# zj15001/PNP_ADMM_CNC_MRI

Hardware: AMD Instinct MI355X
Metric: ADMM iterations/sec on 256x256 complex64 slices (batch=512) (higher is better)
Workload: dtype f32

## Files before the change

pnp_admm_cnc_mri_amd/csrc/kernels_slice256.hip:

```cpp
#include "engine_host.h"
#include "fused_layout.h"
#include "slice_layout.h"
#include <math.h>
#include <stdio.h>
#include <stdlib.h>
#include <vector>

#ifndef SLICE_EARLY
#define SLICE_EARLY 1
#endif
#ifndef SLICE_PRIOSWAP
#define SLICE_PRIOSWAP 1
#endif
#ifndef SLICE_PRIOMASK
#define SLICE_PRIOMASK 6
#endif
#ifndef SLICE_YH_AUX
#define SLICE_YH_AUX 0
#endif
#ifndef SLICE_ST_AUX
#define SLICE_ST_AUX 0
#endif
#ifndef SLICE_RESIDENT
#define SLICE_RESIDENT 1
#endif
#ifndef SLICE_PF
#define SLICE_PF 3
#endif

namespace pnp {

__device__ c32 g_tws[256];

struct SliceArgs {
    float* z;
    float* w;
    float* x;
    const c32* Yh;
    const uint32_t* Mh;
    const c32* Ys;
    const uint32_t* Ms;
    int first, B, iters;
    int slice_xor;
    int flip;
    int state_stride;
    int yh_stride;
    float scale, c;
    ProxParams prox;
    long long* prof;
};

constexpr int RP = 18;
constexpr int REGION = 16 * RP;
constexpr int WREG = 4 * REGION;
constexpr int SL_YS = SL_BUF + REGION;
constexpr int SL_LDS = SL_YS + 256 + 32;
static_assert(SL_WAVES * WREG <= SL_BUF, "wave regions must fit in the buffer they alias");
constexpr int SL4_XB = SL_WAVES * WREG;
constexpr int SL4_YS = SL4_XB + REGION;
constexpr int SL4_RES = SL4_YS + 256 + 32;
constexpr int SL4_LDS = SL4_RES + SL_RES * 256;
static_assert(SL_BUF4 <= SL4_XB && SL4_RES % 2 == 0 && SL4_LDS * 8 <= 160 * 1024, "four-pass LDS map");
template <int PROX> constexpr bool slice_four() { return PROX == 2; }
template <int PROX> constexpr bool slice_res() { return slice_four<PROX>() && SLICE_RESIDENT; }
__device__ __forceinline__ void lds_ld4(const float* p, float (&v)[4]) {
    const float4 q = *reinterpret_cast<const float4*>(p);
    v[0] = q.x; v[1] = q.y; v[2] = q.z; v[3] = q.w;
}
__device__ __forceinline__ void lds_st4(float* p, const float (&v)[4]) { *reinterpret_cast<float4*>(p) = make_float4(v[0], v[1], v[2], v[3]); }

__device__ __forceinline__ void wave_sync() {
    __builtin_amdgcn_fence(__ATOMIC_RELEASE, "wavefront");
    __builtin_amdgcn_wave_barrier();
    __builtin_amdgcn_fence(__ATOMIC_ACQUIRE, "wavefront");
#ifdef SLICE_SYNC_SCHED_BARRIER
    __builtin_amdgcn_sched_barrier(0);
#endif
}

__device__ __forceinline__ void prio_set(int wv, int set) {
#if SLICE_PRIOSWAP
    const bool older_high = (SLICE_PRIOMASK >> set) & 1;
    if (set == 0 || (((SLICE_PRIOMASK >> set) ^ (SLICE_PRIOMASK >> (set - 1))) & 1)) {
        asm volatile("" : "+s"(wv));
        if ((wv < 4) == older_high) __builtin_amdgcn_s_setprio(1); else __builtin_amdgcn_s_setprio(0);
    }
#endif
}

__device__ __forceinline__ int opaque(int v) {
    asm volatile("" : "+v"(v));
    return v;
}
typedef unsigned int u32x4 __attribute__((ext_vector_type(4)));
typedef unsigned int u32x2 __attribute__((ext_vector_type(2)));
typedef __amdgpu_buffer_rsrc_t bufrsrc;
__device__ __forceinline__ bufrsrc make_rsrc(const void* base, unsigned bytes) {
    return __builtin_amdgcn_make_buffer_rsrc(const_cast<void*>(base), 0, (int)bytes, 0x00020000);
}
__device__ __forceinline__ void ld4(bufrsrc r, int voff, int soff, float (&v)[4]) {
    const u32x4 q = __builtin_amdgcn_raw_buffer_load_b128(r, voff, soff, 16);
    v[0] = __uint_as_float(q.x); v[1] = __uint_as_float(q.y); v[2] = __uint_as_float(q.z); v[3] = __uint_as_float(q.w);
}
__device__ __forceinline__ void st4(bufrsrc r, int voff, int soff, const float (&v)[4]) {
    u32x4 q;
    q.x = __float_as_uint(v[0]); q.y = __float_as_uint(v[1]); q.z = __float_as_uint(v[2]); q.w = __float_as_uint(v[3]);
    __builtin_amdgcn_raw_buffer_store_b128(q, r, voff + soff, 0, SLICE_ST_AUX);
}
__device__ __forceinline__ c32 ldc(bufrsrc r, int voff, int soff) {
    const u32x2 q = __builtin_amdgcn_raw_buffer_load_b64(r, voff, soff, 0);
    return mk<float>(__uint_as_float(q.x), __uint_as_float(q.y));
}
struct SliceBufs {
    bufrsrc z, w, x;
    bufrsrc yh, mh, ys, ms;
};

__device__ __forceinline__ void pin(c32& v) { asm volatile("" : "+v"(v.x), "+v"(v.y)); }
__device__ __forceinline__ void mem_fence_compiler() { asm volatile("" ::: "memory"); }

__device__ __forceinline__ float dpp_lane_xor1(float v) {
    return __int_as_float(__builtin_amdgcn_mov_dpp(__float_as_int(v), 0xB1 , 0xF, 0xF, true));
}
__device__ __forceinline__ c32 dpp_lane_xor1(c32 v) { return mk<float>(dpp_lane_xor1(v.x), dpp_lane_xor1(v.y)); }

__device__ __forceinline__ float sub_partner(float a, float b) {
    float r;
    asm("v_subrev_f32_dpp %0, %1, %2 quad_perm:[1,0,3,2] row_mask:0xf bank_mask:0xf bound_ctrl:1" : "=v"(r) : "v"(b), "v"(a));
    return r;
}
__device__ __forceinline__ float add_partner(float a, float b) {
    float r;
    asm("v_add_f32_dpp %0, %1, %2 quad_perm:[1,0,3,2] row_mask:0xf bank_mask:0xf bound_ctrl:1" : "=v"(r) : "v"(b), "v"(a));
    return r;
}

__device__ __forceinline__ float abs_plus(float a, float w) {
    float r;
    asm("v_add_f32_e64 %0, |%1|, %2" : "=v"(r) : "v"(a), "v"(w));
    return r;
}

__device__ __forceinline__ f2 sub2(f2 a, f2 b) {
    f2 r;
    asm("v_pk_add_f32 %0, %1, %2 neg_lo:[0,1] neg_hi:[0,1]" : "=v"(r) : "v"(a), "v"(b));
    return r;
}


template <bool INV>
__device__ __forceinline__ void group_fft256(c32 (&ac)[16], const c32* twl, c32* region, int t) {
    typedef float f4 __attribute__((ext_vector_type(4)));
    const f4* tw4 = reinterpret_cast<const f4*>(twl + RP * t);
    f2* reg2 = reinterpret_cast<f2*>(region);
    f2 a[16];
#pragma unroll
    for (int k = 0; k < 16; ++k) a[k] = to2(ac[k]);
    dft16_pk<INV>(a);
    mem_fence_compiler();
#pragma unroll
    for (int m = 0; m < 4; ++m) {
        const f4 q = tw4[m];
        if (m) a[2 * m] = tmul_v<INV>(a[2 * m], k2(q.x, q.y));
        a[2 * m + 1] = tmul_v<INV>(a[2 * m + 1], k2(q.z, q.w));
    }
    mem_fence_compiler();
#pragma unroll
    for (int m = 4; m < 8; ++m) {
        const f4 q = tw4[m];
        a[2 * m] = tmul_v<INV>(a[2 * m], k2(q.x, q.y));
        a[2 * m + 1] = tmul_v<INV>(a[2 * m + 1], k2(q.z, q.w));
    }
#pragma unroll
    for (int k = 0; k < 16; ++k) reg2[k * RP + t] = a[k];
    wave_sync();
    const f4* row4 = reinterpret_cast<const f4*>(reg2 + t * RP);
#pragma unroll
    for (int m = 0; m < 8; ++m) {
        const f4 q = row4[m];
        a[2 * m] = k2(q.x, q.y);
        a[2 * m + 1] = k2(q.z, q.w);
    }
    wave_sync();
    dft16_pk<INV>(a);
#pragma unroll
    for (int k = 0; k < 16; ++k) ac[k] = from2(a[k]);
}

struct RowLoads {
    float z[8][4], w[8][4];
};
__device__ __forceinline__ int row_set_offset(int set, int wv) { return (32 * set + 4 * wv) * 2048; }
constexpr int ROW_QSTRIDE = 256;

template <int PROX, bool HAS_INV, int Q0, int Q1, bool RESW = false>
__device__ __forceinline__ void issue_row_loads(const SliceBufs& b, RowLoads& L, int soff, int voff, int qbase = 0, const float* resw = nullptr) {
#pragma unroll
    for (int q = qbase + Q0; q < qbase + Q1; ++q) {
        const int vo = voff + ROW_QSTRIDE * q, so = soff;
        if (RESW) {
            ld4(b.z, vo, so, L.z[q]);
            lds_ld4(resw + 64 * q, L.w[q]);
        } else if (PROX == 3) {
            ld4(b.w, vo, so, L.w[q]);
        } else if (PROX != 0 || !HAS_INV) {
            ld4(b.z, vo, so, L.z[q]);
            ld4(b.w, vo, so, L.w[q]);
        }
    }
}

__device__ __forceinline__ f2 clamp2(f2 a, float c) {
    return k2(__builtin_amdgcn_fmed3f(a.x, -c, c), __builtin_amdgcn_fmed3f(a.y, -c, c));
}
__device__ __forceinline__ f2 fma2(f2 a, f2 b, f2 c) { return __builtin_elementwise_fma(a, b, c); }
__device__ __forceinline__ f2 splat(float v) { return k2(v, v); }
template <int PROX>
__device__ __forceinline__ void prox_pair(f2 u, f2& z, f2& w, const ProxParams& pc) {
    if (PROX == 2) {
        const f2 cz = clamp2(z, pc.ib);
        const f2 t = fma2(splat(pc.c1), z, fma2(splat(pc.c2), u, splat(pc.c3) * cz));
        z = t - clamp2(t, pc.thr);
    } else {
        z = u - clamp2(u, pc.thr);
    }
    w = u - z;
}

template <bool HAS_INV, int PROX, bool HAS_FWD, bool RESW = false>
__device__ __forceinline__ void pointwise_q(const SliceBufs& b, const ProxParams& pc, int u_first, bool last,
                                            c32& a0, c32& a1, const float (&z_)[4], const float (&w_)[4], int vs, float* resw = nullptr) {
    f2 z[2] = {k2(z_[0], z_[1]), k2(z_[2], z_[3])}, w[2] = {k2(w_[0], w_[1]), k2(w_[2], w_[3])};
#define SL_X_PLUS(a_, w_) (HAS_INV ? k2(abs_plus((a_).x, (w_).x), abs_plus((a_).y, (w_).y)) : (w_))
#define SL_ST4(buf, v) { const float q_[4] = {v[0].x, v[0].y, v[1].x, v[1].y}; st4(buf, vs, 0, q_); }
    if (PROX == 3) {
        f2 u[2];
#pragma unroll
        for (int jj = 0; jj < 2; ++jj) {
            if (!u_first) {
                asm volatile("");
                w[jj] = w[jj] - (w[jj] - clamp2(w[jj], pc.thr));
            }
            u[jj] = SL_X_PLUS(jj ? a1 : a0, w[jj]);
            z[jj] = u[jj] - clamp2(u[jj], pc.thr);
            w[jj] = u[jj] - z[jj];
        }
        if (!last) {
            SL_ST4(b.w, u);
        } else {
            SL_ST4(b.z, z);
            SL_ST4(b.w, w);
        }
    }
    if (PROX == 1 || PROX == 2) {
#pragma unroll
        for (int jj = 0; jj < 2; ++jj) prox_pair<PROX>(SL_X_PLUS(jj ? a1 : a0, w[jj]), z[jj], w[jj], pc);
        SL_ST4(b.z, z);
        if (RESW) { const float q_[4] = {w[0].x, w[0].y, w[1].x, w[1].y}; lds_st4(resw, q_); }
        else SL_ST4(b.w, w);
    }
#undef SL_ST4
#undef SL_X_PLUS
    if (HAS_FWD) {
        const f2 v0 = sub2(z[0], w[0]), v1 = sub2(z[1], w[1]);
        a0 = from2(v0);
        a1 = from2(v1);
    }
}

__device__ __forceinline__ void store_x_natural(const SliceBufs& b, const c32 (&a)[16], c32* wreg, int set, int wv, int lane) {
    const int g = lane >> 4, t = lane & 15;
    c32* region = wreg + g * REGION;
#pragma unroll
    for (int j = 0; j < 16; ++j) region[t + 16 * j] = mk<float>(fabsf(a[j].x), fabsf(a[j].y));
    wave_sync();
#pragma unroll
    for (int i = 0; i < 4; ++i) {
        const c32* cell = wreg + i * REGION + 4 * lane;
        const float4 c01 = *reinterpret_cast<const float4*>(cell);
        const float4 c23 = *reinterpret_cast<const float4*>(cell + 2);
        const int vs = 16 * lane + (2 * (32 * set + 4 * wv + i)) * 1024;
        const float xa[4] = {c01.x, c01.z, c23.x, c23.z}, xb[4] = {c01.y, c01.w, c23.y, c23.w};
        st4(b.x, vs, 0, xa);
        st4(b.x, vs + 1024, 0, xb);
    }
    wave_sync();
}

#ifndef SLICE_L1_PF
#define SLICE_L1_PF 8
#endif
template <int PROX> constexpr int row_pf() { return (PROX == 3) ? SLICE_L1_PF : SLICE_PF; }
__device__ __forceinline__ float* res_lane(float* res, int wv, int lane) { return res + sl_res_index(4 * wv + (lane >> 4), lane & 15, 0); }
template <int PROX, bool HAS_INV, bool RES = false>
__device__ __forceinline__ void row_phase_prefetch(const SliceBufs& b, RowLoads& L, int wv, int lane, float* res = nullptr) {
    issue_row_loads<PROX, HAS_INV, 0, row_pf<PROX>(), RES>(b, L, row_set_offset(0, wv), 2048 * (lane >> 4) + 16 * (lane & 15), 0, RES ? res_lane(res, wv, lane) : nullptr);
}
template <bool HAS_INV, int PROX, bool HAS_FWD, bool PRELOADED = false, bool RES = false>
__device__ __forceinline__ void row_phase(const SliceBufs& b, const ProxParams& pc, int u_first, bool last, c32 (&F)[SL_SETS][16],
                                          c32* wreg, const c32* twl, int wv, int lane, RowLoads* pre = nullptr, float* res = nullptr) {
    const int g = lane >> 4, t = lane & 15;
    c32* region = wreg + g * REGION;
    const int voff = 2048 * g + 16 * t;
    float* resw = RES ? res_lane(res, wv, lane) : nullptr;
    constexpr bool RES_LOOP = RES && HAS_INV;
    constexpr int PF = row_pf<PROX>();
    RowLoads L;
    if (PRELOADED) L = *pre;
    else issue_row_loads<PROX, HAS_INV, 0, PF, RES_LOOP>(b, L, row_set_offset(0, wv), voff, 0, resw);
#pragma unroll
    for (int set = 0; set < SL_SETS; ++set) {
        c32 (&a)[16] = F[set];
        prio_set(wv, set);
        const int soff = row_set_offset(set, wv);
        if (HAS_INV) {
            group_fft256<true>(a, twl, region, t);
        }
        if (HAS_INV && last) store_x_natural(b, a, wreg, set, wv, lane);
        const int vs = voff + soff;
#pragma unroll
        for (int q = 0; q < 8; ++q) {
            if (RES_LOOP && set == 0) {
                if (q + PF < 8) issue_row_loads<PROX, HAS_INV, 0, 1, true>(b, L, soff, voff, q + PF, resw);
                pointwise_q<HAS_INV, PROX, HAS_FWD, true>(b, pc, u_first, last, a[2 * q], a[2 * q + 1], L.z[q], L.w[q], vs + ROW_QSTRIDE * q, resw + 64 * q);
            } else {
                if (q + PF < 8) issue_row_loads<PROX, HAS_INV, 0, 1>(b, L, soff, voff, q + PF);
                if (RES && !HAS_INV && set == 0) lds_st4(resw + 64 * q, L.w[q]);
                pointwise_q<HAS_INV, PROX, HAS_FWD>(b, pc, u_first, last, a[2 * q], a[2 * q + 1], L.z[q], L.w[q], vs + ROW_QSTRIDE * q);
            }
        }
        if (set + 1 < SL_SETS) issue_row_loads<PROX, HAS_INV, 0, PF>(b, L, row_set_offset(set + 1, wv), voff);
        if (HAS_FWD) {
            group_fft256<false>(a, twl, region, t);
        }
    }
}

__device__ __forceinline__ void resident_flush(const SliceBufs& b, const float* res, int wv, int lane) {
    const float* resw = res_lane(const_cast<float*>(res), wv, lane);
    const int vs = 2048 * (lane >> 4) + 16 * (lane & 15) + row_set_offset(0, wv);
#pragma unroll
    for (int q = 0; q < 8; ++q) {
        float v[4];
        lds_ld4(resw + 64 * q, v);
        st4(b.w, vs + ROW_QSTRIDE * q, 0, v);
    }
}

#define SL_PASS0_REGS(X, t)                                                                       \
    X(0, 0, (t)) X(1, 1, (t) + 16) X(2, 2, (t) + 32) X(3, 3, (t) + 48)                              \
    X(12, 8, ((t) ? SL_M + 64 - (t) : SL_M))                                                      \
    X(13, 13, SL_M + 48 - (t)) X(14, 14, SL_M + 32 - (t)) X(15, 15, SL_M + 16 - (t))
#define SL_PASS1_REGS(X, t)                                                                       \
    X(4, 4, (t)) X(5, 5, (t) + 16) X(6, 6, (t) + 32) X(7, 7, (t) + 48)                              \
    X(8, 12, ((t) ? SL_M + 64 - (t) : SL_M))                                                      \
    X(9, 9, SL_M + 48 - (t)) X(10, 10, SL_M + 32 - (t)) X(11, 11, SL_M + 16 - (t))

#define SL_PASS4_REGS(X, t, Q)                                                                    \
    X(2 * (Q), 2 * (Q), (t)) X(2 * (Q) + 1, 2 * (Q) + 1, (t) + 16)                                  \
    X(14 - 2 * (Q), ((Q) ? 16 - 2 * (Q) : 8), ((t) ? SL_M4 + 32 - (t) : SL_M4))                   \
    X(15 - 2 * (Q), 15 - 2 * (Q), SL_M4 + 16 - (t))

__device__ __forceinline__ void lds_put(c32* p, c32 v, bool swapped) {
    float* f = reinterpret_cast<float*>(p);
    if (swapped) { f[0] = v.y; f[1] = v.x; } else { *p = v; }
}
__device__ __forceinline__ c32 lds_get(const c32* p, bool swapped) {
    const float* f = reinterpret_cast<const float*>(p);
    return swapped ? mk<float>(f[1], f[0]) : *p;
}
template <int P, bool FOUR = false>
__device__ __forceinline__ void t_store_rows(const c32 (&F)[16], c32* rp, int t) {
#define SL_T1_STORE(ja, jb, slot) { lds_put(rp + (slot), t ? F[ja] : F[jb], (ja) >= 8); }
    if (FOUR) { SL_PASS4_REGS(SL_T1_STORE, t, P) } else if (P == 0) { SL_PASS0_REGS(SL_T1_STORE, t) } else { SL_PASS1_REGS(SL_T1_STORE, t) }
#undef SL_T1_STORE
}
template <int P, bool FOUR = false>
__device__ __forceinline__ void t_load_rows(c32 (&F)[16], const c32* rp, int t) {
#define SL_T2_LOAD(ja, jb, slot) { F[ja] = lds_get(rp + (slot), (ja) >= 8); }
    if (FOUR) { SL_PASS4_REGS(SL_T2_LOAD, t, P) } else if (P == 0) { SL_PASS0_REGS(SL_T2_LOAD, t) } else { SL_PASS1_REGS(SL_T2_LOAD, t) }
#undef SL_T2_LOAD
    if (FOUR && P == 3) {
        const c32 a8 = F[8];
        F[8] = t ? a8 : F[14];
        F[14] = t ? F[14] : F[12];
        F[12] = t ? F[12] : F[10];
        F[10] = t ? F[10] : a8;
    }
    if (!FOUR && P == 1) {
        const c32 a0 = F[8];
        F[8] = t ? a0 : F[12];
        F[12] = t ? F[12] : a0;
    }
}

template <bool MAYBE_PACKED, int PITCH = SL_P>
__device__ __forceinline__ void t1_read_col(c32 (&Gs)[16], const c32* buf, int off, int odd, bool packed) {
    int off_hi = off + 64 * PITCH;
    asm volatile("" : "+v"(off_hi));
    const c32 *col = buf + off, *col_hi = buf + off_hi;
#pragma unroll
    for (int jb = 0; jb < 16; jb += 8) {
        c32 own[8];
#pragma unroll
        for (int k = 0; k < 8; ++k) own[k] = jb ? col_hi[8 * k * PITCH] : col[8 * k * PITCH];
#pragma unroll
        for (int k = 0; k < 8; ++k) {
            c32 v = mk<float>(add_partner(own[k].x, own[k].y), sub_partner(own[k].y, own[k].x));
            if (MAYBE_PACKED) {
                const float oy = dpp_lane_xor1(own[k].y);
                const c32 raw = mk<float>(odd ? oy : own[k].x, odd ? own[k].x : oy);
                v = packed ? raw : v;
            }
            Gs[jb + k] = v;
            pin(Gs[jb + k]);
        }
    }
}
template <int P>
__device__ __forceinline__ void t1_pass(const c32 (&F)[SL_SETS][16], c32 (&G)[SL_SETS][16], c32* buf, int wv, int lane) {
    const int g = lane >> 4, t = lane & 15;
#pragma unroll
    for (int set = 0; set < SL_SETS; ++set) t_store_rows<P>(F[set], buf + (32 * set + 4 * wv + g) * SL_P, t);
    __syncthreads();
#pragma unroll
    for (int h = 0; h < 2; ++h) {
        const int cc = 32 * h + 4 * wv + g, odd = t & 1;
        const int off = (t >> 1) * SL_P + cc + (odd ? SL_M : 0);
        if (P == 0 && h == 0 && wv == 0) t1_read_col<true>(G[2 * P + h], buf, off, odd, cc == 0);
        else t1_read_col<false>(G[2 * P + h], buf, off, odd, false);
    }
    __syncthreads();
}

template <bool MAYBE_PACKED, int PITCH = SL_P>
__device__ __forceinline__ void t2_write_col(const c32 (&Gs)[16], c32* buf, int off, int odd, bool packed) {
    int off_hi = off + 64 * PITCH;
    asm volatile("" : "+v"(off_hi));
    c32 *col = buf + off, *col_hi = buf + off_hi;
#pragma unroll
    for (int j = 0; j < 16; ++j) {
        const c32 own = Gs[j];
        c32 v = mk<float>(sub_partner(own.x, own.y), add_partner(own.y, own.x));
        if (MAYBE_PACKED) {
            const c32 other = dpp_lane_xor1(own);
            const c32 raw = mk<float>(odd ? own.y : own.x, odd ? other.y : other.x);
            v = packed ? raw : v;
        }
        if (j < 8) col[8 * j * PITCH] = v; else col_hi[8 * (j - 8) * PITCH] = v;
    }
}
template <int P>
__device__ __forceinline__ void t2_pass(const c32 (&G)[SL_SETS][16], c32 (&F)[SL_SETS][16], c32* buf, int wv, int lane) {
    const int g = lane >> 4, t = lane & 15;
#pragma unroll
    for (int h = 0; h < 2; ++h) {
        const int cc = 32 * h + 4 * wv + g, odd = t & 1;
        const int off = (t >> 1) * SL_P + cc + (odd ? SL_M : 0);
        if (P == 0 && h == 0 && wv == 0) t2_write_col<true>(G[2 * P + h], buf, off, odd, cc == 0);
        else t2_write_col<false>(G[2 * P + h], buf, off, odd, false);
    }
    __syncthreads();
#pragma unroll
    for (int set = 0; set < SL_SETS; ++set) t_load_rows<P>(F[set], buf + (32 * set + 4 * wv + g) * SL_P, t);
    __syncthreads();
}

template <int Q>
__device__ __forceinline__ void t1_pass4(const c32 (&F)[SL_SETS][16], c32 (&G)[SL_SETS][16], c32* buf, int wv, int lane) {
    const int g = lane >> 4, t = lane & 15;
#pragma unroll
    for (int set = 0; set < SL_SETS; ++set) t_store_rows<Q, true>(F[set], buf + (32 * set + 4 * wv + g) * SL_P4, t);
    __syncthreads();
    const int cc = 4 * wv + g, odd = t & 1;
    const int off = (t >> 1) * SL_P4 + cc + (odd ? SL_M4 : 0);
    if (Q == 0 && wv == 0) t1_read_col<true, SL_P4>(G[Q], buf, off, odd, cc == 0);
    else t1_read_col<false, SL_P4>(G[Q], buf, off, odd, false);
    __syncthreads();
}
template <int Q>
__device__ __forceinline__ void t2_pass4(const c32 (&G)[SL_SETS][16], c32 (&F)[SL_SETS][16], c32* buf, int wv, int lane) {
    const int g = lane >> 4, t = lane & 15;
    const int cc = 4 * wv + g, odd = t & 1;
    const int off = (t >> 1) * SL_P4 + cc + (odd ? SL_M4 : 0);
    if (Q == 0 && wv == 0) t2_write_col<true, SL_P4>(G[Q], buf, off, odd, cc == 0);
    else t2_write_col<false, SL_P4>(G[Q], buf, off, odd, false);
    __syncthreads();
#pragma unroll
    for (int set = 0; set < SL_SETS; ++set) t_load_rows<Q, true>(F[set], buf + (32 * set + 4 * wv + g) * SL_P4, t);
    __syncthreads();
}

struct ColLoads {
    c32 yh[16];
    uint32_t code;
};
__device__ __forceinline__ void issue_col_loads(const SliceBufs& b, ColLoads& Y, int set, int wv, int lane) {
    const int ybase = (set * 8 + wv) * 8192;
    Y.code = __builtin_amdgcn_raw_buffer_load_b32(b.mh, 4 * lane, (set * 8 + wv) * 64 * 4, 0);
#pragma unroll
    for (int jp = 0; jp < 8; ++jp) {
        const u32x4 q = __builtin_amdgcn_raw_buffer_load_b128(b.yh, 16 * lane + 1024 * (jp & 3), ybase + 4096 * (jp >> 2), SLICE_YH_AUX);
        Y.yh[2 * jp] = mk<float>(__uint_as_float(q.x), __uint_as_float(q.y));
        Y.yh[2 * jp + 1] = mk<float>(__uint_as_float(q.z), __uint_as_float(q.w));
    }
}

__device__ __forceinline__ float code_byte(unsigned m, int byte) {
    float r;
    if (byte == 0) asm("v_cvt_f32_ubyte0 %0, %1" : "=v"(r) : "v"(m));
    else if (byte == 1) asm("v_cvt_f32_ubyte1 %0, %1" : "=v"(r) : "v"(m));
    else if (byte == 2) asm("v_cvt_f32_ubyte2 %0, %1" : "=v"(r) : "v"(m));
    else asm("v_cvt_f32_ubyte3 %0, %1" : "=v"(r) : "v"(m));
    return r;
}
__device__ __forceinline__ void blend_set(c32 (&a)[16], const c32 (&yh)[16], unsigned code, float cs, float chs, float os) {
    const unsigned m[4] = {code & 0x03030303u, (code >> 2) & 0x03030303u, (code >> 4) & 0x03030303u, (code >> 6) & 0x03030303u};
#pragma unroll
    for (int j = 0; j < 16; j += 2) {
        const f2 cf = k2(code_byte(m[j & 3], j >> 2), code_byte(m[(j & 3) + 1], j >> 2));
        const f2 A2 = fma2(splat(-chs), cf, splat(os));
        a[j] = from2(fma2(A2.xx, to2(a[j]), splat(cs) * to2(yh[j])));
        a[j + 1] = from2(fma2(A2.yy, to2(a[j + 1]), splat(cs) * to2(yh[j + 1])));
    }
}

__device__ __forceinline__ void col_phase(const SliceBufs& b, float cdc, float scale, c32 (&G)[SL_SETS][16], c32* wreg, c32* ysl, const c32* twl, int wv, int lane) {
    const int g = lane >> 4, t = lane & 15;
    c32* region = wreg + g * REGION;
    const float cs = cdc * scale, chs = 0.5f * cdc * scale;
    ColLoads Y;
    issue_col_loads(b, Y, 0, wv, lane);
    if (wv == 0) {
        __builtin_amdgcn_raw_ptr_buffer_load_lds(b.ys, ysl, 16, 16 * lane, 0, 0, 0);
        __builtin_amdgcn_raw_ptr_buffer_load_lds(b.ys, ysl + 128, 16, 16 * lane, 1024, 0, 0);
        __builtin_amdgcn_raw_ptr_buffer_load_lds(b.ms, ysl + 256, 4, 4 * lane, 0, 0, 0);
    }
#pragma unroll
    for (int set = 0; set < SL_SETS; ++set) {
        c32 (&a)[16] = G[set];
        prio_set(wv, set);
        group_fft256<false>(a, twl, region, t);
        if (set == 0 && wv == 0 && g == 0) {
#pragma unroll
            for (int j = 0; j < 16; ++j) region[t + 16 * j] = a[j];
            region[256 + t] = a[0];
            wave_sync();
            const uint32_t code_b = reinterpret_cast<const uint32_t*>(ysl + 256)[t];
            const c32* mirror = region + (16 - t);
            const unsigned ma[4] = {Y.code & 0x03030303u, (Y.code >> 2) & 0x03030303u, (Y.code >> 4) & 0x03030303u, (Y.code >> 6) & 0x03030303u};
            const unsigned mb[4] = {code_b & 0x03030303u, (code_b >> 2) & 0x03030303u, (code_b >> 4) & 0x03030303u, (code_b >> 6) & 0x03030303u};
#pragma unroll
            for (int j = 0; j < 16; ++j) {
                const c32 gm = mirror[16 * (15 - j)];
                const c32 A = blend_scaled_f(unpack_a(a[j], gm), Y.yh[j], code_byte(ma[j & 3], j >> 2), cs, chs, scale);
                const c32 Bv = blend_scaled_f(unpack_b(a[j], gm), ysl[t + 16 * j], code_byte(mb[j & 3], j >> 2), cs, chs, scale);
                a[j] = repack_p(A, Bv);
            }
            wave_sync();
        } else {
            blend_set(a, Y.yh, Y.code, cs, 0.5f * chs, 0.5f * scale);
        }
        if (set + 1 < SL_SETS) issue_col_loads(b, Y, set + 1, wv, lane);
        group_fft256<true>(a, twl, region, t);
    }
}

template <int PROX>
__global__ __launch_bounds__(512) void k_slice(SliceArgs p) {
    constexpr bool FOUR = slice_four<PROX>(), RES = slice_res<PROX>();
    __shared__ __attribute__((aligned(16))) c32 lds[FOUR ? SL4_LDS : SL_LDS];
    const int tid = threadIdx.x, lane = tid & 63;
    const int wv = __builtin_amdgcn_readfirstlane(tid >> 6);
    c32* twl = lds + (FOUR ? SL4_XB : SL_BUF);
    c32* ysl = lds + (FOUR ? SL4_YS : SL_YS);
    float* res = RES ? reinterpret_cast<float*>(lds + SL4_RES) : nullptr;
    if (tid < 256) twl[RP * (tid >> 4) + (tid & 15)] = g_tws[((tid >> 4) * (tid & 15)) & 255];
    c32* wreg = lds + wv * WREG;
    __syncthreads();
    for (int sb = blockIdx.x; sb < p.B; sb += gridDim.x) {
        const int sx = ((sb ^ p.slice_xor) < p.B) ? (sb ^ p.slice_xor) : sb;
        const int slice = p.first + (p.flip ? p.B - 1 - sx : sx);
        const size_t so = (size_t)slice * p.state_stride;
        SliceBufs b;
        b.z = make_rsrc(p.z + so, 65536 * 4); b.w = make_rsrc(p.w + so, 65536 * 4); b.x = make_rsrc(p.x + (size_t)slice * 65536, 65536 * 4);
        b.yh = make_rsrc(p.Yh + (size_t)slice * p.yh_stride, YH3_SLICE * 8); b.mh = make_rsrc(p.Mh + (size_t)slice * MH3_SLICE, MH3_SLICE * 4);
        b.ys = make_rsrc(p.Ys + (size_t)slice * 256, 256 * 8); b.ms = make_rsrc(p.Ms + (size_t)slice * 16, 16 * 4);
        c32 F[SL_SETS][16];
#ifdef SLICE_PROF
        long long* prof = (p.prof && tid == 0 && sb == (int)blockIdx.x) ? p.prof + (size_t)slice * (2 + 6 * p.iters) : nullptr;
#define SL_STAMP() if (prof) *prof++ = wall_clock64()
#else
#define SL_STAMP()
#endif
        SL_STAMP();
        row_phase<false, 0, true, false, RES>(b, p.prox, 1, false, F, wreg, twl, wv, opaque(lane), nullptr, res);
        SL_STAMP();
        for (int it = 0; it < p.iters; ++it) {
            c32 G[SL_SETS][16];
            __syncthreads();
            SL_STAMP();
            if (FOUR) {
                t1_pass4<0>(F, G, lds, wv, opaque(lane));
                t1_pass4<1>(F, G, lds, wv, opaque(lane));
                t1_pass4<2>(F, G, lds, wv, opaque(lane));
                t1_pass4<3>(F, G, lds, wv, opaque(lane));
            } else {
                t1_pass<0>(F, G, lds, wv, opaque(lane));
                t1_pass<1>(F, G, lds, wv, opaque(lane));
            }
#ifdef SLICE_PROF_CLOCK
            if (prof) *prof++ = (long long)__builtin_readcyclecounter();
#else
            SL_STAMP();
#endif
            col_phase(b, p.c, p.scale, G, wreg, ysl, twl, wv, opaque(lane));
            SL_STAMP();
            __syncthreads();
            SL_STAMP();
            if (FOUR) {
                t2_pass4<0>(G, F, lds, wv, opaque(lane));
                t2_pass4<1>(G, F, lds, wv, opaque(lane));
                t2_pass4<2>(G, F, lds, wv, opaque(lane));
            } else {
                t2_pass<0>(G, F, lds, wv, opaque(lane));
            }
#if SLICE_EARLY
            RowLoads L0;
            row_phase_prefetch<PROX, true, RES>(b, L0, wv, opaque(lane), res);
#endif
            if (FOUR) t2_pass4<3>(G, F, lds, wv, opaque(lane));
            else t2_pass<1>(G, F, lds, wv, opaque(lane));
            SL_STAMP();
            const int u_first = (it == 0);
#if SLICE_EARLY
            row_phase<true, PROX, true, true, RES>(b, p.prox, u_first, it + 1 == p.iters, F, wreg, twl, wv, opaque(lane), &L0, res);
#else
            row_phase<true, PROX, true, false, RES>(b, p.prox, u_first, it + 1 == p.iters, F, wreg, twl, wv, opaque(lane), nullptr, res);
#endif
            SL_STAMP();
        }
        if (RES) resident_flush(b, res, wv, opaque(lane));
        __syncthreads();
    }
}

constexpr int SP_P = 17;
__global__ __launch_bounds__(256) void k_sprepare(const c32* y, const uint8_t* mask_bank, const int32_t* mask_id,
                                                  c32* Yh, uint32_t* Mh, c32* Ys, uint32_t* Ms, int yh_stride) {
    __shared__ c32 yd[256 * SP_P], ym[256 * SP_P];
    __shared__ uint8_t md[256 * SP_P], mm[256 * SP_P];
    const int tid = threadIdx.x, m = blockIdx.x, slice = blockIdx.y;
    const int mid = mask_id ? mask_id[slice] : 0;
    const c32* ys = y + (size_t)slice * 65536;
    const uint8_t* ms = mask_bank + (size_t)mid * 65536;
    const int ncol = (m == 8) ? 1 : 16;
#pragma unroll 4
    for (int i = 0; i < 16; ++i) {
        const int idx = tid + 256 * i, r = idx >> 4, c = idx & 15;
        if (c < ncol) {
            const int k2 = 16 * m + c, k2m = (256 - k2) & 255;
            yd[r * SP_P + c] = ys[r * 256 + k2];
            md[r * SP_P + c] = ms[r * 256 + k2];
            ym[r * SP_P + c] = ys[r * 256 + k2m];
            mm[r * SP_P + c] = ms[r * 256 + k2m];
        }
    }
    __syncthreads();
    auto entry = [&](int k1, int c, c32& yh) -> int {
        const int r2 = (256 - k1) & 255;
        const int m1 = md[k1 * SP_P + c] != 0, m2 = mm[r2 * SP_P + c] != 0;
        const c32 y1 = yd[k1 * SP_P + c], y2 = ym[r2 * SP_P + c];
        yh = mk<float>(0.5f * ((m1 ? y1.x : 0.f) + (m2 ? y2.x : 0.f)), 0.5f * ((m1 ? y1.y : 0.f) - (m2 ? y2.y : 0.f)));
        return m1 + m2;
    };
    if (m == 8) {
        c32 yh;
        const int code = entry(tid, 0, yh);
        Ys[(size_t)slice * 256 + tid] = yh;
        __shared__ int codes[256];
        codes[tid] = code;
        __syncthreads();
        if (tid < 16) {
            uint32_t v = 0;
#pragma unroll
            for (int jj = 0; jj < 16; ++jj) v |= (uint32_t)codes[tid + 16 * jj] << (2 * jj);
            Ms[slice * 16 + tid] = v;
        }
        return;
    }
    const int set = m >> 1;
#pragma unroll 4
    for (int i = 0; i < 16; ++i) {
        const int o = tid + 256 * i, blk = o >> 10, e = o & 1023;
        const int jp = e >> 7, lane = (e >> 1) & 63, j = 2 * jp + (e & 1);
        const int g = lane >> 4, t = lane & 15, wv = 4 * (m & 1) + blk;
        c32 yh;
        (void)entry(t + 16 * j, 4 * blk + g, yh);
        Yh[(size_t)slice * yh_stride + yh3_index(0, set, j, wv, lane)] = yh;
    }
    {
        const int blk = tid >> 6, lane = tid & 63, g = lane >> 4, t = lane & 15, wv = 4 * (m & 1) + blk;
        uint32_t v = 0;
#pragma unroll
        for (int j = 0; j < 16; ++j) {
            c32 yh;
            v |= (uint32_t)entry(t + 16 * j, 4 * blk + g, yh) << (2 * j);
        }
        Mh[mh3_index(slice, set, wv, lane)] = v;
    }
}

template <bool TO_SLICE>
__global__ __launch_bounds__(128) void k_state_order(const float* sz, const float* sw, float* dz, float* dw, int src_stride, int dst_stride) {
    __shared__ float tile[2][2048];
    const size_t sbase = (size_t)blockIdx.y * src_stride + (size_t)blockIdx.x * 2048, dbase = (size_t)blockIdx.y * dst_stride + (size_t)blockIdx.x * 2048;
    const float4* pz = reinterpret_cast<const float4*>(sz + sbase);
    const float4* pw = reinterpret_cast<const float4*>(sw + sbase);
    float4* qz = reinterpret_cast<float4*>(dz + dbase);
    float4* qw = reinterpret_cast<float4*>(dw + dbase);
    float4 vz[4], vw[4];
#pragma unroll
    for (int u = 0; u < 4; ++u) { vz[u] = pz[threadIdx.x + 128 * u]; vw[u] = pw[threadIdx.x + 128 * u]; }
#pragma unroll
    for (int u = 0; u < 4; ++u) {
        const int i = threadIdx.x + 128 * u, row = i >> 6, n0 = 4 * (i & 63);
        const float az[4] = {vz[u].x, vz[u].y, vz[u].z, vz[u].w}, aw[4] = {vw[u].x, vw[u].y, vw[u].z, vw[u].w};
#pragma unroll
        for (int k = 0; k < 4; ++k) {
            const int at = TO_SLICE ? (int)sl_state_index(row, n0 + k) : 4 * i + k;
            tile[0][at] = az[k];
            tile[1][at] = aw[k];
        }
    }
    __syncthreads();
#pragma unroll
    for (int u = 0; u < 4; ++u) {
        const int i = threadIdx.x + 128 * u, row = i >> 6, n0 = 4 * (i & 63);
        float oz[4], ow[4];
#pragma unroll
        for (int k = 0; k < 4; ++k) {
            const int at = TO_SLICE ? 4 * i + k : (int)sl_state_index(row, n0 + k);
            oz[k] = tile[0][at];
            ow[k] = tile[1][at];
        }
        qz[i] = make_float4(oz[0], oz[1], oz[2], oz[3]);
        qw[i] = make_float4(ow[0], ow[1], ow[2], ow[3]);
    }
}

struct Slice256 {
    int Bmax = 0, cus = 0;
    int flip = 0;
    int pad = 0, yh_pad = 0;
    float* zs = nullptr;
    float* ws = nullptr;
    c32* Yh = nullptr;
    uint32_t* Mh = nullptr;
    c32* Ys = nullptr;
    uint32_t* Ms = nullptr;
    SideQueues queues;
};

int slice256_cus(const Slice256* f) { return f && f->cus > 0 ? f->cus : 256; }

hipError_t slice256_state_order(Slice256* f, hipStream_t s, float* z, float* w, int B, bool to_slice) {
    if (B <= 0) return hipSuccess;
    if (f && f->pad > 0) {
        if (to_slice) hipLaunchKernelGGL(k_state_order<true>, dim3(32, B), dim3(128), 0, s, z, w, f->zs, f->ws, 65536, 65536 + f->pad);
        else          hipLaunchKernelGGL(k_state_order<false>, dim3(32, B), dim3(128), 0, s, f->zs, f->ws, z, w, 65536 + f->pad, 65536);
    } else {
        if (to_slice) hipLaunchKernelGGL(k_state_order<true>, dim3(32, B), dim3(128), 0, s, z, w, z, w, 65536, 65536);
        else          hipLaunchKernelGGL(k_state_order<false>, dim3(32, B), dim3(128), 0, s, z, w, z, w, 65536, 65536);
    }
    return hipGetLastError();
}

void slice256_destroy(Slice256* f) {
    if (!f) return;
    if (f->zs) (void)hipFree(f->zs);
    if (f->ws) (void)hipFree(f->ws);
    if (f->Yh) (void)hipFree(f->Yh);
    if (f->Mh) (void)hipFree(f->Mh);
    if (f->Ys) (void)hipFree(f->Ys);
    if (f->Ms) (void)hipFree(f->Ms);
    delete f;
}

Slice256* slice256_create(int Bmax, int pad_kb, int yh_pad_kb, hipError_t* err) {
    Slice256* f = new Slice256();
    f->Bmax = Bmax;
    f->pad = (pad_kb > 0 ? pad_kb : 0) * 256;
    f->yh_pad = (yh_pad_kb > 0 ? yh_pad_kb : 0) * 128;
    hipError_t e = hipMalloc((void**)&f->Yh, (size_t)Bmax * (YH3_SLICE + f->yh_pad) * sizeof(c32));
    if (e == hipSuccess && f->pad > 0) e = hipMalloc((void**)&f->zs, (size_t)Bmax * (65536 + f->pad) * sizeof(float));
    if (e == hipSuccess && f->pad > 0) e = hipMalloc((void**)&f->ws, (size_t)Bmax * (65536 + f->pad) * sizeof(float));
    if (e == hipSuccess) e = hipMalloc((void**)&f->Mh, (size_t)Bmax * MH3_SLICE * sizeof(uint32_t));
    if (e == hipSuccess) e = hipMalloc((void**)&f->Ys, (size_t)Bmax * 256 * sizeof(c32));
    if (e == hipSuccess) e = hipMalloc((void**)&f->Ms, (size_t)Bmax * 16 * sizeof(uint32_t));
    if (e == hipSuccess) e = upload_twiddle_table<float>(HIP_SYMBOL(g_tws), 256);
    if (e == hipSuccess) {
        int dev = 0;
        hipDeviceProp_t prop;
        e = hipGetDevice(&dev);
        if (e == hipSuccess) e = hipGetDeviceProperties(&prop, dev);
        if (e == hipSuccess) f->cus = prop.multiProcessorCount;
    }
    if (e != hipSuccess) {
        slice256_destroy(f);
        *err = e;
        return nullptr;
    }
    *err = hipSuccess;
    return f;
}

hipError_t slice256_prepare(Slice256* f, hipStream_t s, const float2* y, const uint8_t* mask_bank, const int32_t* mask_id, int B) {
    if (B > f->Bmax) return hipErrorInvalidValue;
    hipLaunchKernelGGL(k_sprepare, dim3(9, B), dim3(256), 0, s, reinterpret_cast<const c32*>(y), mask_bank, mask_id,
                       f->Yh, f->Mh, f->Ys, f->Ms, (int)YH3_SLICE + f->yh_pad);
    return hipGetLastError();
}

static hipError_t launch_slice(hipStream_t s, const SliceArgs& a, int prox) {
    const dim3 grid(a.B);
    if (prox == 2)      hipLaunchKernelGGL(k_slice<2>, grid, dim3(512), 0, s, a);
    else if (prox == 1) hipLaunchKernelGGL(k_slice<1>, grid, dim3(512), 0, s, a);
    else                hipLaunchKernelGGL(k_slice<3>, grid, dim3(512), 0, s, a);
    return hipGetLastError();
}

hipError_t slice256_run(Slice256* f, hipStream_t s, float* z, float* w, float* x, int B, int iters, bool cnc, float dc_c,
                        ProxParams pp, const FusedSchedule& sch) {
    if (iters <= 0) return hipSuccess;
    SliceArgs a;
    a.z = f->pad > 0 ? f->zs : z; a.w = f->pad > 0 ? f->ws : w; a.x = x; a.Yh = f->Yh;
    a.state_stride = 65536 + f->pad; a.yh_stride = (int)YH3_SLICE + f->yh_pad; a.Mh = f->Mh; a.Ys = f->Ys; a.Ms = f->Ms;
    a.first = 0; a.B = B; a.iters = iters; a.scale = 1.0f / 65536.0f; a.c = dc_c;
    a.prox = pp;
    a.prof = nullptr;
    a.flip = 0;
    a.slice_xor = sch.slice_xor;
    if (a.slice_xor < 0 || (B & (B - 1)) != 0 || a.slice_xor >= B) a.slice_xor = 0;
    const int prox = prox_kind(cnc, sch);
    int segments = sch.slice_segment > 0 ? (iters + sch.slice_segment - 1) / sch.slice_segment : 1;
    if (segments < 1) segments = 1;

    long long* d_prof = nullptr;
#ifdef SLICE_PROF
    const char* prof_path = getenv("PNP_SLICE_PROF");
#else
    const char* prof_path = nullptr;
#endif
    const LoopPlan plan = plan_slice(B, prof_path ? FusedSchedule{} : sch);
    const size_t prof_n = (size_t)B * (2 + 6 * (size_t)iters);
    if (prof_path) {
        segments = 1;
        if (hipMalloc((void**)&d_prof, prof_n * sizeof(long long)) == hipSuccess) {
            (void)hipMemsetAsync(d_prof, 0, prof_n * sizeof(long long), s);
            a.prof = d_prof;
        }
    }
    if (!prof_path && B > slice256_cus(f) && sch.slice_flip) { a.flip = f->flip; f->flip ^= 1; }
    const hipError_t e = run_parts(f->queues, s, plan, B, [&](hipStream_t sq, const Part& p) {
        hipError_t r = hipSuccess;
        int done = 0;
        for (int g = 0; g < segments && r == hipSuccess; ++g) {
            const int n = (iters - done + (segments - g) - 1) / (segments - g);
            a.first = p.first; a.B = p.count; a.iters = n;
            r = launch_slice(sq, a, prox);
            done += n;
        }
        return r;
    });
    if (d_prof) {
        std::vector<long long> h(prof_n);
        (void)hipStreamSynchronize(s);
        (void)hipMemcpy(h.data(), d_prof, prof_n * sizeof(long long), hipMemcpyDeviceToHost);
        (void)hipFree(d_prof);
        if (FILE* fo = fopen(prof_path, "wb")) {
            const int hdr[2] = {B, iters};
            fwrite(hdr, sizeof(int), 2, fo);
            fwrite(h.data(), sizeof(long long), prof_n, fo);
            fclose(fo);
        }
    }
    return e;
}

}
```

pnp_admm_cnc_mri_amd/csrc/slice_layout.h:

```cpp
#pragma once
#include <stddef.h>
#include <stdint.h>
#include "fft16.h"

namespace pnp {

constexpr int SL_P = 132;
constexpr int SL_M = 66;
constexpr int SL_BUF = 128 * SL_P;

PNP_HD int sl_pass(int k) { return (k < 64 || k > 192 || k == 128) ? 0 : 1; }
PNP_HD int sl_slot(int k) {
    if (k < 64) return k;
    if (k == 128) return SL_M;
    if (k > 192) return SL_M + 256 - k;
    if (k < 128) return k - 64;
    return SL_M + 192 - k;
}
constexpr int SL_P4 = 68;
constexpr int SL_M4 = 34;
constexpr int SL_BUF4 = 128 * SL_P4;
PNP_HD int sl_pass4(int k) { return k == 128 ? 0 : k < 128 ? (k >> 5) : ((256 - k) >> 5); }
PNP_HD int sl_slot4(int k) { return k == 128 ? SL_M4 : k < 128 ? (k & 31) : SL_M4 + ((256 - k) & 31); }
constexpr int SL_RES = 32;
PNP_HD int sl_res_index(int r, int t, int q) { return 512 * r + 64 * q + 4 * t; }

constexpr int SL_WAVES = 8, SL_SETS = 4;
PNP_HD int sl_unit(int set, int wv, int lane) { return 32 * set + 4 * wv + (lane >> 4); }

constexpr size_t YH3_SLICE = 4 * 16 * 8 * 64;
constexpr size_t MH3_SLICE = 4 * 8 * 64;
PNP_HD size_t yh3_index(int slice, int set, int j, int wv, int lane) {
    return (size_t)slice * YH3_SLICE + ((((size_t)set * 8 + wv) * 8 + (j >> 1)) * 64 + lane) * 2 + (j & 1);
}
PNP_HD size_t mh3_index(int slice, int set, int wv, int lane) { return (size_t)slice * MH3_SLICE + (((size_t)set * 8 + wv) * 64 + lane); }

PNP_HD size_t sl_state_index(int row, int n) {
    return (size_t)(row >> 1) * 512 + 64 * (n >> 5) + 4 * (n & 15) + 2 * ((n >> 4) & 1) + (row & 1);
}


}
```

Before: 10850.

## Keep more of the w state resident in LDS and registers across ADMM iterations

Generalizes the resident-w scheme from set 0 only to a per-(set, q) home map. Each w chunk lives in LDS, in registers, or in HBM, chosen by compile-time unit masks. By default two more units of set 1 go to a second LDS region and two units of set 3 are held in registers. This cuts global w load and store traffic per iteration, at the cost of extra LDS footprint and register pressure, which may reduce occupancy or cause spills.

```diff
diff --git a/pnp_admm_cnc_mri_amd/csrc/kernels_slice256.hip b/pnp_admm_cnc_mri_amd/csrc/kernels_slice256.hip
--- a/pnp_admm_cnc_mri_amd/csrc/kernels_slice256.hip
+++ b/pnp_admm_cnc_mri_amd/csrc/kernels_slice256.hip
@@ -20,9 +20,6 @@
 #endif
 #ifndef SLICE_ST_AUX
 #define SLICE_ST_AUX 0
-#endif
-#ifndef SLICE_RESIDENT
-#define SLICE_RESIDENT 1
 #endif
 #ifndef SLICE_PF
 #define SLICE_PF 3
@@ -59,7 +56,8 @@
 constexpr int SL4_XB = SL_WAVES * WREG;
 constexpr int SL4_YS = SL4_XB + REGION;
 constexpr int SL4_RES = SL4_YS + 256 + 32;
-constexpr int SL4_LDS = SL4_RES + SL_RES * 256;
+__device__ __forceinline__ int sl_lds_float(int set, int q) { return set == 0 ? sl_res_index(0, 0, q) : sl_res1_index(popc8(sl_units_lds(set) & ((1u << q) - 1)), 0, 0); }
+constexpr int SL4_LDS = SL4_RES + SL_RES * 256 + SL_NLDS1 * 1024;
 static_assert(SL_BUF4 <= SL4_XB && SL4_RES % 2 == 0 && SL4_LDS * 8 <= 160 * 1024, "four-pass LDS map");
 template <int PROX> constexpr bool slice_four() { return PROX == 2; }
 template <int PROX> constexpr bool slice_res() { return slice_four<PROX>() && SLICE_RESIDENT; }
@@ -194,13 +192,14 @@
 constexpr int ROW_QSTRIDE = 256;
 
 template <int PROX, bool HAS_INV, int Q0, int Q1, bool RESW = false>
-__device__ __forceinline__ void issue_row_loads(const SliceBufs& b, RowLoads& L, int soff, int voff, int qbase = 0, const float* resw = nullptr) {
+__device__ __forceinline__ void issue_row_loads(const SliceBufs& b, RowLoads& L, int soff, int voff, int qbase = 0, int set = 0, const float* resl = nullptr) {
 #pragma unroll
     for (int q = qbase + Q0; q < qbase + Q1; ++q) {
         const int vo = voff + ROW_QSTRIDE * q, so = soff;
-        if (RESW) {
+        const int home = RESW ? w_home(set, q) : W_HBM;
+        if (home != W_HBM) {
             ld4(b.z, vo, so, L.z[q]);
-            lds_ld4(resw + 64 * q, L.w[q]);
+            if (home == W_LDS) lds_ld4(resl + sl_lds_float(set, q), L.w[q]);
         } else if (PROX == 3) {
             ld4(b.w, vo, so, L.w[q]);
         } else if (PROX != 0 || !HAS_INV) {
@@ -227,9 +226,10 @@
     w = u - z;
 }
 
-template <bool HAS_INV, int PROX, bool HAS_FWD, bool RESW = false>
+template <bool HAS_INV, int PROX, bool HAS_FWD>
 __device__ __forceinline__ void pointwise_q(const SliceBufs& b, const ProxParams& pc, int u_first, bool last,
-                                            c32& a0, c32& a1, const float (&z_)[4], const float (&w_)[4], int vs, float* resw = nullptr) {
+                                            c32& a0, c32& a1, const float (&z_)[4], const float (&w_)[4], int vs,
+                                            int home = W_HBM, float* resw = nullptr, float* wq = nullptr) {
     f2 z[2] = {k2(z_[0], z_[1]), k2(z_[2], z_[3])}, w[2] = {k2(w_[0], w_[1]), k2(w_[2], w_[3])};
 #define SL_X_PLUS(a_, w_) (HAS_INV ? k2(abs_plus((a_).x, (w_).x), abs_plus((a_).y, (w_).y)) : (w_))
 #define SL_ST4(buf, v) { const float q_[4] = {v[0].x, v[0].y, v[1].x, v[1].y}; st4(buf, vs, 0, q_); }
@@ -256,7 +256,8 @@
 #pragma unroll
         for (int jj = 0; jj < 2; ++jj) prox_pair<PROX>(SL_X_PLUS(jj ? a1 : a0, w[jj]), z[jj], w[jj], pc);
         SL_ST4(b.z, z);
-        if (RESW) { const float q_[4] = {w[0].x, w[0].y, w[1].x, w[1].y}; lds_st4(resw, q_); }
+        if (home == W_LDS) { const float q_[4] = {w[0].x, w[0].y, w[1].x, w[1].y}; lds_st4(resw, q_); }
+        else if (home == W_REG) { wq[0] = w[0].x; wq[1] = w[0].y; wq[2] = w[1].x; wq[3] = w[1].y; }
         else SL_ST4(b.w, w);
     }
 #undef SL_ST4
@@ -291,23 +292,26 @@
 #define SLICE_L1_PF 8
 #endif
 template <int PROX> constexpr int row_pf() { return (PROX == 3) ? SLICE_L1_PF : SLICE_PF; }
-__device__ __forceinline__ float* res_lane(float* res, int wv, int lane) { return res + sl_res_index(4 * wv + (lane >> 4), lane & 15, 0); }
+__device__ __forceinline__ float* res_lane(float* res, int set, int wv, int lane) {
+    return set == 0 ? res + sl_res_index(4 * wv + (lane >> 4), lane & 15, 0) : res + SL_RES * 512 + sl_res1_index(0, 4 * wv + (lane >> 4), lane & 15);
+}
+typedef float ResRegs[SL_NREG > 0 ? SL_NREG : 1][4];
 template <int PROX, bool HAS_INV, bool RES = false>
 __device__ __forceinline__ void row_phase_prefetch(const SliceBufs& b, RowLoads& L, int wv, int lane, float* res = nullptr) {
-    issue_row_loads<PROX, HAS_INV, 0, row_pf<PROX>(), RES>(b, L, row_set_offset(0, wv), 2048 * (lane >> 4) + 16 * (lane & 15), 0, RES ? res_lane(res, wv, lane) : nullptr);
+    issue_row_loads<PROX, HAS_INV, 0, row_pf<PROX>(), RES>(b, L, row_set_offset(0, wv), 2048 * (lane >> 4) + 16 * (lane & 15), 0, 0, RES ? res_lane(res, 0, wv, lane) : nullptr);
 }
 template <bool HAS_INV, int PROX, bool HAS_FWD, bool PRELOADED = false, bool RES = false>
 __device__ __forceinline__ void row_phase(const SliceBufs& b, const ProxParams& pc, int u_first, bool last, c32 (&F)[SL_SETS][16],
-                                          c32* wreg, const c32* twl, int wv, int lane, RowLoads* pre = nullptr, float* res = nullptr) {
+                                          c32* wreg, const c32* twl, int wv, int lane, ResRegs& wr, RowLoads* pre = nullptr, float* res = nullptr) {
     const int g = lane >> 4, t = lane & 15;
     c32* region = wreg + g * REGION;
     const int voff = 2048 * g + 16 * t;
-    float* resw = RES ? res_lane(res, wv, lane) : nullptr;
+    float* const resl[2] = {RES ? res_lane(res, 0, wv, lane) : nullptr, RES && SL_NLDS1 ? res_lane(res, 1, wv, lane) : nullptr};
     constexpr bool RES_LOOP = RES && HAS_INV;
     constexpr int PF = row_pf<PROX>();
     RowLoads L;
     if (PRELOADED) L = *pre;
-    else issue_row_loads<PROX, HAS_INV, 0, PF, RES_LOOP>(b, L, row_set_offset(0, wv), voff, 0, resw);
+    else issue_row_loads<PROX, HAS_INV, 0, PF, RES_LOOP>(b, L, row_set_offset(0, wv), voff, 0, 0, resl[0]);
 #pragma unroll
     for (int set = 0; set < SL_SETS; ++set) {
         c32 (&a)[16] = F[set];
@@ -320,30 +324,41 @@
         const int vs = voff + soff;
 #pragma unroll
         for (int q = 0; q < 8; ++q) {
-            if (RES_LOOP && set == 0) {
-                if (q + PF < 8) issue_row_loads<PROX, HAS_INV, 0, 1, true>(b, L, soff, voff, q + PF, resw);
-                pointwise_q<HAS_INV, PROX, HAS_FWD, true>(b, pc, u_first, last, a[2 * q], a[2 * q + 1], L.z[q], L.w[q], vs + ROW_QSTRIDE * q, resw + 64 * q);
+            const int home = RES ? w_home(set, q) : W_HBM;
+            float* const rl = home == W_LDS ? resl[set] + sl_lds_float(set, q) : nullptr;
+            float* const wq = wr[home == W_REG ? sl_reg_slot(set, q) : 0];
+            if (q + PF < 8) issue_row_loads<PROX, HAS_INV, 0, 1, RES_LOOP>(b, L, soff, voff, q + PF, set, resl[set < 2 ? set : 0]);
+            if (RES_LOOP && home != W_HBM) {
+                pointwise_q<HAS_INV, PROX, HAS_FWD>(b, pc, u_first, last, a[2 * q], a[2 * q + 1], L.z[q], home == W_REG ? wr[sl_reg_slot(set, q)] : L.w[q],
+                                                    vs + ROW_QSTRIDE * q, home, rl, wq);
             } else {
-                if (q + PF < 8) issue_row_loads<PROX, HAS_INV, 0, 1>(b, L, soff, voff, q + PF);
-                if (RES && !HAS_INV && set == 0) lds_st4(resw + 64 * q, L.w[q]);
+                if (home == W_LDS) lds_st4(rl, L.w[q]);
+                if (home == W_REG) { wq[0] = L.w[q][0]; wq[1] = L.w[q][1]; wq[2] = L.w[q][2]; wq[3] = L.w[q][3]; }
                 pointwise_q<HAS_INV, PROX, HAS_FWD>(b, pc, u_first, last, a[2 * q], a[2 * q + 1], L.z[q], L.w[q], vs + ROW_QSTRIDE * q);
             }
         }
-        if (set + 1 < SL_SETS) issue_row_loads<PROX, HAS_INV, 0, PF>(b, L, row_set_offset(set + 1, wv), voff);
+        if (set + 1 < SL_SETS) issue_row_loads<PROX, HAS_INV, 0, PF, RES_LOOP>(b, L, row_set_offset(set + 1, wv), voff, 0, set + 1, resl[set + 1 < 2 ? set + 1 : 0]);
         if (HAS_FWD) {
             group_fft256<false>(a, twl, region, t);
         }
     }
 }
 
-__device__ __forceinline__ void resident_flush(const SliceBufs& b, const float* res, int wv, int lane) {
-    const float* resw = res_lane(const_cast<float*>(res), wv, lane);
-    const int vs = 2048 * (lane >> 4) + 16 * (lane & 15) + row_set_offset(0, wv);
-#pragma unroll
-    for (int q = 0; q < 8; ++q) {
-        float v[4];
-        lds_ld4(resw + 64 * q, v);
-        st4(b.w, vs + ROW_QSTRIDE * q, 0, v);
+__device__ __forceinline__ void resident_flush(const SliceBufs& b, float* res, const ResRegs& wr, int wv, int lane) {
+#pragma unroll
+    for (int set = 0; set < SL_SETS; ++set) {
+        const int vs = 2048 * (lane >> 4) + 16 * (lane & 15) + row_set_offset(set, wv);
+#pragma unroll
+        for (int q = 0; q < 8; ++q) {
+            const int home = w_home(set, q);
+            if (home == W_LDS) {
+                float v[4];
+                lds_ld4(res_lane(res, set, wv, lane) + sl_lds_float(set, q), v);
+                st4(b.w, vs + ROW_QSTRIDE * q, 0, v);
+            } else if (home == W_REG) {
+                st4(b.w, vs + ROW_QSTRIDE * q, 0, wr[sl_reg_slot(set, q)]);
+            }
+        }
     }
 }
 
@@ -587,6 +602,7 @@
         b.yh = make_rsrc(p.Yh + (size_t)slice * p.yh_stride, YH3_SLICE * 8); b.mh = make_rsrc(p.Mh + (size_t)slice * MH3_SLICE, MH3_SLICE * 4);
         b.ys = make_rsrc(p.Ys + (size_t)slice * 256, 256 * 8); b.ms = make_rsrc(p.Ms + (size_t)slice * 16, 16 * 4);
         c32 F[SL_SETS][16];
+        ResRegs wres;
 #ifdef SLICE_PROF
         long long* prof = (p.prof && tid == 0 && sb == (int)blockIdx.x) ? p.prof + (size_t)slice * (2 + 6 * p.iters) : nullptr;
 #define SL_STAMP() if (prof) *prof++ = wall_clock64()
@@ -594,7 +610,7 @@
 #define SL_STAMP()
 #endif
         SL_STAMP();
-        row_phase<false, 0, true, false, RES>(b, p.prox, 1, false, F, wreg, twl, wv, opaque(lane), nullptr, res);
+        row_phase<false, 0, true, false, RES>(b, p.prox, 1, false, F, wreg, twl, wv, opaque(lane), wres, nullptr, res);
         SL_STAMP();
         for (int it = 0; it < p.iters; ++it) {
             c32 G[SL_SETS][16];
@@ -634,13 +650,13 @@
             SL_STAMP();
             const int u_first = (it == 0);
 #if SLICE_EARLY
-            row_phase<true, PROX, true, true, RES>(b, p.prox, u_first, it + 1 == p.iters, F, wreg, twl, wv, opaque(lane), &L0, res);
+            row_phase<true, PROX, true, true, RES>(b, p.prox, u_first, it + 1 == p.iters, F, wreg, twl, wv, opaque(lane), wres, &L0, res);
 #else
-            row_phase<true, PROX, true, false, RES>(b, p.prox, u_first, it + 1 == p.iters, F, wreg, twl, wv, opaque(lane), nullptr, res);
+            row_phase<true, PROX, true, false, RES>(b, p.prox, u_first, it + 1 == p.iters, F, wreg, twl, wv, opaque(lane), wres, nullptr, res);
 #endif
             SL_STAMP();
         }
-        if (RES) resident_flush(b, res, wv, opaque(lane));
+        if (RES) resident_flush(b, res, wres, wv, opaque(lane));
         __syncthreads();
     }
 }
diff --git a/pnp_admm_cnc_mri_amd/csrc/slice_layout.h b/pnp_admm_cnc_mri_amd/csrc/slice_layout.h
--- a/pnp_admm_cnc_mri_amd/csrc/slice_layout.h
+++ b/pnp_admm_cnc_mri_amd/csrc/slice_layout.h
@@ -22,10 +22,34 @@
 constexpr int SL_BUF4 = 128 * SL_P4;
 PNP_HD int sl_pass4(int k) { return k == 128 ? 0 : k < 128 ? (k >> 5) : ((256 - k) >> 5); }
 PNP_HD int sl_slot4(int k) { return k == 128 ? SL_M4 : k < 128 ? (k & 31) : SL_M4 + ((256 - k) & 31); }
+constexpr int SL_WAVES = 8, SL_SETS = 4;
 constexpr int SL_RES = 32;
 PNP_HD int sl_res_index(int r, int t, int q) { return 512 * r + 64 * q + 4 * t; }
+constexpr int SL_RES1 = 2;
+PNP_HD int sl_res1_index(int u, int rr, int t) { return 2048 * u + 64 * rr + 4 * t; }
+#ifndef SLICE_RESIDENT
+#define SLICE_RESIDENT 1
+#endif
+#ifndef SLICE_UNITS_LDS1
+#define SLICE_UNITS_LDS1 0x03
+#endif
+#ifndef SLICE_UNITS_REG
+#define SLICE_UNITS_REG 0x03000000
+#endif
+constexpr int popc8(unsigned m) { int n = 0; for (int i = 0; i < 8; ++i) n += (m >> i) & 1; return n; }
+constexpr unsigned sl_units_lds(int set) { return SLICE_RESIDENT == 0 ? 0u : set == 0 ? 0xFFu : (SLICE_RESIDENT == 1 && set == 1) ? (SLICE_UNITS_LDS1 & 0xFFu) : 0u; }
+constexpr unsigned sl_units_reg(int set) { return SLICE_RESIDENT == 1 && set < SL_SETS ? ((unsigned)SLICE_UNITS_REG >> (8 * set)) & 0xFFu & ~sl_units_lds(set) : 0u; }
+enum { W_HBM = 0, W_LDS = 1, W_REG = 2 };
+constexpr int w_home(int set, int q) { return ((sl_units_lds(set) >> q) & 1) ? W_LDS : ((sl_units_reg(set) >> q) & 1) ? W_REG : W_HBM; }
+constexpr int sl_reg_slot(int set, int q) {
+    int n = 0;
+    for (int s = 0; s < set; ++s) n += popc8(sl_units_reg(s));
+    return n + (set < SL_SETS ? popc8(sl_units_reg(set) & ((1u << q) - 1)) : 0);
+}
+constexpr int SL_NREG = sl_reg_slot(SL_SETS, 0);
+constexpr int SL_NLDS1 = popc8(sl_units_lds(1));
+static_assert(SL_NLDS1 <= SL_RES1, "the second resident region holds SL_RES1 units");
 
-constexpr int SL_WAVES = 8, SL_SETS = 4;
 PNP_HD int sl_unit(int set, int wv, int lane) { return 32 * set + 4 * wv + (lane >> 4); }
 
 constexpr size_t YH3_SLICE = 4 * 16 * 8 * 64;
```

Result: faster. 11140 (median of 6 runs) (+2.7%).
